# mjrgh/DCSExplorer

Measured on AMD Instinct MI355X. Metric: bit_exact_int16_pcm_samples_per_sec, higher is better.
Workload: dtype int16; 1 GPU; survey3_65536; gpu_max_hw_queues=4, samples_per_frame=240, frames_per_wave=8, wavefronts_per_launch=8192, arithmetic=ADSP-2105 1.15 fixed point, 32-bit integer intermediates, partition=range over streams, no collective, scale=1, inflight=1, frames_per_chunk=all, full=False

## Files before the change

dcsexplorer_amd/csrc/dcs_common.h:

```cpp
#pragma once
#include <stdint.h>
#include <stddef.h>
#include "../../include/dcs_hip.h"

#define DCS_CB94_TOTAL   940
#define DCS_TRIE94_MAX   64
#define DCS_TRIE93_MAX   128

struct DcsLdsTables
{
    uint16_t cb94[DCS_CB94_TOTAL];
    uint16_t fast93[256];
    uint16_t trie93[DCS_TRIE93_MAX];
    uint16_t bandBits93a[64];
    uint16_t scaleCb93a[80];
    uint8_t  inputs93a[24];
    uint16_t raw94[20];
    uint32_t band94[72];
    uint16_t scale64[64];
    uint8_t  padDecode_[8];
    uint16_t cbInfo[8];
    uint16_t xlat94[48];
    uint8_t  preAdj94[32];
    uint16_t scaleMant[4];
    uint8_t  pad_[8];
};
#define DCS_LDS_DECODE_BYTES 3424
#define DCS_B94_RAW      (1u << 21)
#define DCS_B94_ZERO     (1u << 22)
#define DCS_B94_STOP     (1u << 23)
#define DCS_B94_FATAL    (1u << 24)
#define DCS_B94_TYPE0    51

#define DCS_LANE_CONSTS 24
#define DCS_K94_PRE   0
#define DCS_K94_TWB   8
#define DCS_K94_OVLA  22
#define DCS_K94_OVLB  23
#define DCS_K93_TWB   0
#define DCS_K93_OVL   15

struct DcsDevTables
{
    DcsLdsTables lds;
    uint32_t lane94[64][DCS_LANE_CONSTS];
    uint32_t lane93[64][DCS_LANE_CONSTS];
    uint16_t fast94[256];
    uint16_t trie94[DCS_TRIE94_MAX];
    uint16_t pair93a[2048];
    uint16_t fftCoef[256];
    uint16_t ovlCoef[16];
    int32_t  twA[8][4];
    uint8_t  multi94[6][1 << 10];
};
#define DCS_IDX_MULTI_BITS 10
#define DCS_IDX_MULTI_SAMPLES 4

const DcsDevTables &dcsTables();

int dcsFrameScaleV(const uint16_t *vol, uint16_t *mixMul, const uint8_t *counted, int nch);

#define DCS_POOL_DW_PER_FRAME 56
#define DCS_POOL_DW_MIN       320
#define DCS_MAX_FRAME_BITS    4480

#ifdef __cplusplus
static inline
#ifdef __HIPCC__
__host__ __device__
#endif
uint32_t dcsPoolDwords(uint64_t streamOff, uint32_t hdrLen, uint32_t bitOff, uint32_t nBits)
{
    const uint32_t inDword = static_cast<uint32_t>(((streamOff + 2 + hdrLen) * 8 + bitOff) & 31);
    return (inDword + nBits + 31) / 32 + 3;
}
#endif

#ifdef __cplusplus
static inline
// ... 205 lines not shown
```

dcsexplorer_amd/csrc/dcs_decode_chunk.inc.h:

```cpp
    DCS_STAMP(1);

    struct { uint32_t job; uint32_t prevSlot, flags, nSrc, shiftXform; uint32_t firstSrc, prevJob, poolOff, bpl; } slot;
    uint32_t exportNext;
    uint4 pd0, pd1, phdr;
    uint2 pd2;
    {
        uint4 *scratch = reinterpret_cast<uint4 *>(L.pool());
        static_assert(kHeadVec * 16 <= poolDwords(FPW) * 4, "the package head fits in the bit pool");
        if (lane < kHeadVec)
            scratch[lane] = phead0;
        if (kHeadLoads > 1 && lane + 64 < kHeadVec)
            scratch[lane + 64] = phead1;
        waveSync();
        const uint4 *sp5 = scratch + 5 * s;
        const uint4 s0 = sp5[0];
        pd0 = sp5[1]; pd1 = sp5[2];
        const uint4 d2v = sp5[3];
        pd2 = make_uint2(d2v.x, d2v.y);
        phdr = sp5[4];
        waveSync();
        slot.job = s0.x;
        slot.prevSlot = s0.y & 0xFFu; slot.flags = (s0.y >> 8) & 0xFFu; slot.nSrc = (s0.y >> 16) & 0xFFu; slot.shiftXform = s0.y >> 24;
        slot.firstSrc = s0.z; slot.prevJob = s0.w;
        slot.poolOff = d2v.z & 0xFFFFu;
// ... 326 lines not shown
        }
        const int lpfShift = (xf == DCS_XFORM_94) ? 3 : 4;
        const int g = lane >> lpfShift;
        const bool active = g < n;
        const int mySlot = s0 + (active ? g : 0);
        const int myWord = __shfl(slotWord, mySlot);
        const int myFlags = myWord & 0xFF, myPrevSlot = (myWord >> 8) & 0xFF, myShift = myWord >> 16;
        const uint32_t myJob = static_cast<uint32_t>(__shfl(slotJob, mySlot));
        const uint32_t myPrevJob = static_cast<uint32_t>(__shfl(jobPrev, mySlot));
        const int lr = (xf == DCS_XFORM_94) ? bitrevN(lane & 7, 3) : bitrevN(lane & 15, 4);

        uint32_t extTail = 0;
        if (__any(active && (myFlags & DCS_SLOT_EXT_TAIL) != 0))
        {
            if (active && (myFlags & DCS_SLOT_EXT_TAIL) != 0 && a.tailsIn != nullptr)
            {
                const size_t k = static_cast<size_t>(myPrevJob & 0x7FFFFFFFu);
                extTail = (xf == DCS_XFORM_94) ? reinterpret_cast<const uint32_t *>(a.tailsIn)[k * 8 + lr]
                                               : static_cast<uint32_t>(static_cast<uint16_t>(a.tailsIn[k * 16 + lr]));
            }
        }

        PassLane P;
        P.rowC = active ? reinterpret_cast<uint32_t *>(L.row(mySlot)) : L.pool();
#ifdef DCS_STAMPS_XFORM
        P.stamp = stamp;
#endif
        P.l = lane & ((1 << lpfShift) - 1);
        P.shiftPair = static_cast<uint32_t>(myShift) * 0x00010001u;
        P.paced = paced && kPace.steps && s0 + n >= nSlots;

        uint32_t x[16];
        BflyRegs R;
        R.k8000 = 0x8000u; R.k10000 = 0x10000u; R.watch = 0xFFFFu;
        R.k4000 = 0x4000u; R.watchB = 0x7FFF7FFFu;
        asm volatile("" : "+v"(R.k8000), "+v"(R.k10000), "+v"(R.k4000));
        if (xf == DCS_XFORM_94)
            transform94x8<kPace.levels>(P, W, C, R, x);
        else
            transform93x4<kPace.levels>(P, W, C, R, x);
        if (s0 == 0) DCS_STAMP(14);

        {
            const int ts = active ? mySlot : FPW;
            if (xf == DCS_XFORM_94)
                tails[ts * 8 + lr] = x[15];
            else
                reinterpret_cast<uint16_t *>(tails)[ts * 16 + lr] = static_cast<uint16_t>(x[15]);
        }
        waveSync();

        if (s0 == 0) DCS_STAMP(15);
        const bool emit = active && !(myFlags & DCS_SLOT_HALO);
        const bool hasPrev = myPrevSlot != DCS_NO_PREV_SLOT;
        const bool exporter = active && (myFlags & DCS_SLOT_EXPORT) != 0;
        const bool deferred = active && (myFlags & DCS_SLOT_IMPORT) != 0;
#ifndef DCS_RDV_SPLIT_FPW4
#define DCS_RDV_SPLIT_FPW4 12
#endif
        constexpr int kSplit = FPW == 4 ? DCS_RDV_SPLIT_FPW4 : 8;
        int lrA = lr;
        if (FPW == 4)
            asm volatile("" : "+v"(lrA));
        unsigned long long metAsProducer = 0, metAsConsumer = 0;
        auto rendezvous = [&](uint32_t mine0, uint32_t tailOut)
        {
            if (exporter)
                metAsProducer = __hip_atomic_exchange(a.handoff + static_cast<size_t>(chunk) * 16 + lrA, handoffWord(a.epoch, 0u, tailOut),
                                                      __ATOMIC_RELAXED, __HIP_MEMORY_SCOPE_AGENT);
            if (deferred)
                metAsConsumer = __hip_atomic_exchange(a.handoff + static_cast<size_t>(myPrevJob) * 16 + lrA, handoffWord(a.epoch, 1u, mine0),
                                                      __ATOMIC_RELAXED, __HIP_MEMORY_SCOPE_AGENT);
        };
        if (xf == DCS_XFORM_94)
        {
            uint32_t tailPair = tails[(hasPrev ? myPrevSlot : mySlot) * 8 + lr];
            tailPair = hasPrev ? tailPair : extTail;
            const uint32_t mixed = packC(overlapMix(reC(x[0]), C.k[DCS_K94_OVLA] & 0xFFFFu, reC(tailPair), C.k[DCS_K94_OVLB] & 0xFFFFu),
                                         overlapMix(imC(x[0]), C.k[DCS_K94_OVLA] >> 16, imC(tailPair), C.k[DCS_K94_OVLB] >> 16));
            x[0] = deferred ? x[0] : mixed;
            uint32_t *out = reinterpret_cast<uint32_t *>(a.pcm) + static_cast<size_t>(myJob) * (DCS_FRAME_SAMPLES / 2) + lrA;
            if (emit)
            {
                if (!deferred)
                    out[0] = x[0];
#pragma unroll
                for (int r = 1 ; r < kSplit ; ++r)
                    out[8 * bitrevN(r, 4)] = x[r];
            }
            rendezvous(x[0], x[15]);
            if (emit)
            {
#pragma unroll
                for (int r = kSplit ; r < 15 ; ++r)
                    out[8 * bitrevN(r, 4)] = x[r];
                if (a.tailsOut != nullptr && (myFlags & DCS_SLOT_KEEP_TAIL))
// ... 52 lines not shown
```

dcsexplorer_amd/csrc/dcs_kernels.hip.h:

```cpp
#pragma once
#include <hip/hip_runtime.h>
#include <type_traits>
#include <cstddef>
#include "dcs_common.h"

namespace dcsk {

struct Stamper
{
#ifdef DCS_STAMPS
    unsigned long long *p;
#ifdef DCS_STAMPS_REALTIME
    __device__ __forceinline__ void operator()(int k) const { if (p != nullptr) p[k] = __builtin_amdgcn_s_memrealtime(); }
#else
    __device__ __forceinline__ void operator()(int k) const { if (p != nullptr) p[k] = __builtin_amdgcn_s_memtime(); }
#endif
#else
    __device__ __forceinline__ void operator()(int) const { }
#endif
};
#define DCS_STAMP(k) stamp(k)

__device__ __forceinline__ unsigned long long handoffWord(uint32_t epoch, uint32_t who, uint32_t payload)
{
// ... 643 lines not shown
    mr = odd ? mrOdd : mr;
    exponent = ((exponent + (odd ? 1 : 0)) >> 1) + 1;
    const uint32_t up = mr << (exponent & 31);
    const uint32_t down = static_cast<uint32_t>(static_cast<int>(mr) >> ((-exponent) & 31));
    uint32_t ar = (exponent >= 0 ? up : down) >> 16;
    ar = neg ? static_cast<uint32_t>(-sx16(ar)) & 0xFFFFu : ar;
    ar = x != 0 ? ar : 0u;
    *reinterpret_cast<uint32_t *>(row) = ar;
}

typedef short s16x2 __attribute__((ext_vector_type(2)));
typedef unsigned short u16x2 __attribute__((ext_vector_type(2)));

__device__ __forceinline__ uint32_t pkAddSat(uint32_t a, uint32_t b)
{ return __builtin_bit_cast(uint32_t, __builtin_elementwise_add_sat(__builtin_bit_cast(s16x2, a), __builtin_bit_cast(s16x2, b))); }
__device__ __forceinline__ uint32_t pkSubSat(uint32_t a, uint32_t b)
{ return __builtin_bit_cast(uint32_t, __builtin_elementwise_sub_sat(__builtin_bit_cast(s16x2, a), __builtin_bit_cast(s16x2, b))); }
__device__ __forceinline__ uint32_t pkAdd(uint32_t a, uint32_t b)
{ return __builtin_bit_cast(uint32_t, static_cast<u16x2>(__builtin_bit_cast(u16x2, a) + __builtin_bit_cast(u16x2, b))); }
__device__ __forceinline__ uint32_t pkSub(uint32_t a, uint32_t b)
{ return __builtin_bit_cast(uint32_t, static_cast<u16x2>(__builtin_bit_cast(u16x2, a) - __builtin_bit_cast(u16x2, b))); }
__device__ __forceinline__ uint32_t pkAshr(uint32_t a, uint32_t shiftPair)
{ return __builtin_bit_cast(uint32_t, static_cast<s16x2>(__builtin_bit_cast(s16x2, a) >> __builtin_bit_cast(s16x2, shiftPair))); }

__device__ __forceinline__ uint32_t packC(int re, int im) { return (static_cast<uint32_t>(re) & 0xFFFFu) | (static_cast<uint32_t>(im) << 16); }
__device__ __forceinline__ int reC(uint32_t c) { return sx16(c); }
__device__ __forceinline__ int imC(uint32_t c) { return static_cast<int>(c) >> 16; }

__device__ __forceinline__ void quirkWatch(uint32_t &watch, uint32_t a, uint32_t b)
{
    asm("v_min_u16 %0, %0, %1\n\tv_min_u16 %0, %0, %2" : "+v"(watch) : "v"(a), "v"(b));
}
__device__ __forceinline__ bool quirkSeen(uint32_t watch) { return __any((watch & 0xFFFFu) == 0); }
#define DCS_MUL_SEL(dst, x, xsel, y, ysel) \
    asm("v_mul_i32_i24_sdwa %0, sext(%1), sext(%2) dst_sel:DWORD dst_unused:UNUSED_PAD src0_sel:" xsel " src1_sel:" ysel : "=v"(dst) : "v"(x), "v"(y))

struct BflyRegs
{
    uint32_t k8000, k10000; uint32_t watch;
    uint32_t k4000, watchB;
};

struct TwScalar { int c2, s2, ns2; };
struct TwA { TwScalar t[8]; };
constexpr int kTwADoubled[8][2] = { { -65536, 0 }, { 0, -65536 }, { -46340, -46340 }, { 46340, -46340 },
                                    { -60548, -25080 }, { 25080, -60548 }, { -25080, -60548 }, { 60548, -25080 } };
__device__ __forceinline__ void loadTwA(const DcsDevTables *, TwA &W)
{
#pragma unroll
    for (int k = 2 ; k < 8 ; ++k)
        W.t[k] = TwScalar{ kTwADoubled[k][0], kTwADoubled[k][1], -kTwADoubled[k][1] };
}

__device__ __forceinline__ uint32_t rotateExact(uint32_t A, int c, int s)
{
    const int are = reC(A), aim = imC(A);
    const int p2 = __mul24(aim, s);
    const int dR = __mul24(are, c) - p2;
    const int q2 = __mul24(are, s);
    const int dI = __mul24(aim, c) + q2;
    uint32_t mrR = (static_cast<uint32_t>(dR) << 1) + 0x8000u;
    uint32_t mrI = (static_cast<uint32_t>(dI) << 1) + 0x8000u;
    if ((p2 & 0x7FFF) == 0x4000) mrR &= ~0x10000u;
    if ((q2 & 0x7FFF) == 0x4000) mrI &= ~0x10000u;
    return __builtin_amdgcn_perm(mrI, mrR, 0x07060302u);
}

__device__ __forceinline__ uint32_t rotateFastA(uint32_t A, const TwScalar &t, BflyRegs &R)
{
    const int are = reC(A), aim = imC(A);
    const uint32_t nP = static_cast<uint32_t>(__mul24(aim, t.ns2)) + R.k8000;
    const uint32_t mrR = static_cast<uint32_t>(__mul24(are, t.c2)) + nP;
    const uint32_t qK = static_cast<uint32_t>(__mul24(are, t.s2)) + R.k8000;
    const uint32_t mrI = static_cast<uint32_t>(__mul24(aim, t.c2)) + qK;
    quirkWatch(R.watch, nP, qK);
    return __builtin_amdgcn_perm(mrI, mrR, 0x07060302u);
}
__device__ __forceinline__ uint32_t shl1Add(uint32_t a, uint32_t b)
{
    uint32_t r = (a << 1) + b;
    asm("" : "+v"(r));
    return r;
}
template <bool TIGHT>
__device__ __forceinline__ uint32_t rotateFastB(uint32_t A, uint32_t tw, BflyRegs &R)
{
    int p1, p2, q1, q2;
    DCS_MUL_SEL(p2, A, "WORD_1", tw, "WORD_1");
    DCS_MUL_SEL(p1, A, "WORD_0", tw, "WORD_0");
    DCS_MUL_SEL(q2, A, "WORD_0", tw, "WORD_1");
    DCS_MUL_SEL(q1, A, "WORD_1", tw, "WORD_0");
    if (TIGHT)
    {
        const uint32_t tR = shl1Add(static_cast<uint32_t>(p2), R.k8000);
        const uint32_t mrR = shl1Add(static_cast<uint32_t>(p1), R.k10000) - tR;
        const uint32_t qK = shl1Add(static_cast<uint32_t>(q2), R.k8000);
        const uint32_t mrI = shl1Add(static_cast<uint32_t>(q1), qK);
        quirkWatch(R.watch, tR, qK);
        return __builtin_amdgcn_perm(mrI, mrR, 0x07060302u);
    }
    const uint32_t mrR = (static_cast<uint32_t>(p1 - p2) << 1) + R.k8000;
    const uint32_t qK = (static_cast<uint32_t>(q2) << 1) + R.k8000;
    const uint32_t mrI = (static_cast<uint32_t>(q1) << 1) + qK;
    quirkWatch(R.watch, (static_cast<uint32_t>(p2) << 1) + R.k8000, qK);
    return __builtin_amdgcn_perm(mrI, mrR, 0x07060302u);
}

struct TwDot { uint32_t re, im, s2; };
__device__ __forceinline__ TwDot deriveTwDot(uint32_t tw)
{
    TwDot d;
    d.im = __builtin_amdgcn_alignbit(tw, tw, 16);
    d.re = __builtin_bit_cast(uint32_t, static_cast<u16x2>(__builtin_bit_cast(u16x2, tw) * __builtin_bit_cast(u16x2, 0xFFFF0001u)));
    asm("v_pk_add_u16 %0, %1, %1 op_sel:[1,1] op_sel_hi:[1,1]" : "=v"(d.s2) : "v"(tw));
    return d;
}
template <bool FIX>
__device__ __forceinline__ uint32_t rotateDotB(uint32_t A, const TwDot &t, BflyRegs &R, uint32_t fixMask)
{
    uint32_t xR, xI, lows;
    const uint32_t cR = FIX ? ((A & fixMask) | R.k4000) : R.k4000;
    asm("v_dot2_i32_i16 %0, %1, %2, %3" : "=v"(xR) : "v"(A), "v"(t.re), "v"(cR));
    asm("v_dot2_i32_i16 %0, %1, %2, %3" : "=v"(xI) : "v"(A), "v"(t.im), "v"(R.k4000));
    asm("v_pk_mul_lo_u16 %0, %1, %2" : "=v"(lows) : "v"(A), "v"(t.s2));
    asm("v_pk_min_i16 %0, %0, %1" : "+v"(R.watchB) : "v"(lows));
    return __builtin_amdgcn_perm(xI << 1, xR << 1, 0x07060302u);
}
__device__ __forceinline__ bool quirkSeenB(uint32_t w) { return __any((w & 0xFFFFu) == 0x8000u || (w >> 16) == 0x8000u); }

template <bool SAT>
__device__ __forceinline__ void addSub(uint32_t u, uint32_t T, uint32_t &lo, uint32_t &hi)
{
    if (SAT) { lo = pkSubSat(u, T); hi = pkAddSat(u, T); }
    else     { lo = pkSub(u, T);    hi = pkAdd(u, T); }
}

__device__ __forceinline__ uint32_t rotateByMinusOne(uint32_t A) { return pkSub(0u, A); }
__device__ __forceinline__ uint32_t rotateByMinusI(uint32_t A)
{
    return __builtin_bit_cast(uint32_t, static_cast<u16x2>(__builtin_bit_cast(u16x2, __builtin_amdgcn_alignbit(A, A, 16))
                                                            * __builtin_bit_cast(u16x2, 0xFFFF0001u)));
}

template <bool SAT, int D, int SH>
__device__ __forceinline__ void stageA(uint32_t (&x)[16], const TwA &W, BflyRegs &R)
{
    uint32_t y[16];
#pragma unroll
    for (int r = 0 ; r < 16 ; ++r)
        if (!(r & D))
        {
            const int idx = r >> SH;
            const uint32_t T = idx == 0 ? rotateByMinusOne(x[r + D]) : idx == 1 ? rotateByMinusI(x[r + D])
                                                                                 : rotateFastA(x[r + D], W.t[idx], R);
            addSub<SAT>(x[r], T, y[r], y[r + D]);
        }
    if (__builtin_expect(quirkSeen(R.watch), 0))
    {
        R.watch = 0xFFFFu;
#pragma unroll
        for (int r = 0 ; r < 16 ; ++r)
            if (!(r & D) && (r >> SH) >= 2)
            {
                int c2 = W.t[r >> SH].c2, s2 = W.t[r >> SH].s2;
                asm volatile("" : "+v"(c2), "+v"(s2));
                addSub<SAT>(x[r], rotateExact(x[r + D], c2 >> 1, s2 >> 1), y[r], y[r + D]);
            }
    }
#pragma unroll
    for (int r = 0 ; r < 16 ; ++r)
        x[r] = y[r];
}
template <bool SAT, int D, int SH, bool DOT = !SAT>
__device__ __forceinline__ void stageB(uint32_t (&x)[16], const uint32_t *tw, BflyRegs &R)
{
    uint32_t y[16];
    bool redo;
    if constexpr (DOT)
    {
        constexpr int kTw = 8 / D;
        TwDot td[kTw];
#pragma unroll
        for (int k = 0 ; k < kTw ; ++k)
            td[k] = deriveTwDot(tw[k]);
        constexpr int kFix = kTw == 1 ? 0 : 1;
        const uint32_t fixMask = tw[kFix] == 0x80000000u ? 0xFFFF0000u : 0u;
#pragma unroll
        for (int r = 0 ; r < 16 ; ++r)
            if (!(r & D))
            {
                const uint32_t T = (r >> SH) == kFix ? rotateDotB<true>(x[r + D], td[r >> SH], R, fixMask)
                                                     : rotateDotB<false>(x[r + D], td[r >> SH], R, 0u);
                addSub<SAT>(x[r], T, y[r], y[r + D]);
            }
        redo = quirkSeenB(R.watchB);
        if (redo)
            R.watchB = 0x7FFF7FFFu;
    }
    else
    {
#pragma unroll
        for (int r = 0 ; r < 16 ; ++r)
            if (!(r & D))
                addSub<SAT>(x[r], rotateFastB<SAT>(x[r + D], tw[r >> SH], R), y[r], y[r + D]);
        redo = quirkSeen(R.watch);
        if (redo)
            R.watch = 0xFFFFu;
    }
    if (__builtin_expect(redo, 0))
    {
#pragma unroll
        for (int r = 0 ; r < 16 ; ++r)
            if (!(r & D))
                addSub<SAT>(x[r], rotateExact(x[r + D], sx16(tw[r >> SH]), static_cast<int>(tw[r >> SH]) >> 16), y[r], y[r + D]);
    }
#pragma unroll
    for (int r = 0 ; r < 16 ; ++r)
        x[r] = y[r];
}

__device__ __forceinline__ int bitrev9(int v) { return static_cast<int>(__brev(static_cast<uint32_t>(v)) >> 23); }
__device__ __forceinline__ int bitrevN(int v, int bits) { return static_cast<int>(__brev(static_cast<uint32_t>(v)) >> (32 - bits)); }

__device__ __forceinline__ int overlapMix(int x, uint32_t cx, int o, uint32_t co)
{
    const uint32_t a = static_cast<uint32_t>(x * static_cast<int>(cx)) << 1;
    const uint32_t b = static_cast<uint32_t>(o * static_cast<int>(co)) << 1;
    return static_cast<int>(a + b + 0x8000u) >> 16;
}

typedef uint32_t u32x4a4 __attribute__((ext_vector_type(4), aligned(4)));

struct LaneConsts { uint32_t k[DCS_LANE_CONSTS]; };
__device__ __forceinline__ void loadLaneConsts(const DcsDevTables *G, int lane, int xform, LaneConsts &C)
{
    const uint4 *src = reinterpret_cast<const uint4 *>(xform == DCS_XFORM_94 ? G->lane94[lane] : G->lane93[lane]);
#pragma unroll
    for (int i = 0 ; i < DCS_LANE_CONSTS / 4 ; ++i)
    {
        const uint4 v = src[i];
        C.k[4 * i] = v.x; C.k[4 * i + 1] = v.y; C.k[4 * i + 2] = v.z; C.k[4 * i + 3] = v.w;
    }
}

__device__ __forceinline__ void waveSync()
{
    __builtin_amdgcn_fence(__ATOMIC_RELEASE, "wavefront");
    __builtin_amdgcn_wave_barrier();
    __builtin_amdgcn_fence(__ATOMIC_ACQUIRE, "wavefront");
}

struct PassLane
{
    uint32_t *rowC;
    int l;
    uint32_t shiftPair;
    bool paced;
#ifdef DCS_STAMPS_XFORM
    Stamper stamp;
#endif
};
constexpr int kPaceSteps = 2 | (1 << 2) | (0 << 4);
#define DCS_PACE_STEP(k) do { if (P.paced) __builtin_amdgcn_s_setprio((STEPS >> (2 * (k))) & 3); } while (0)
#ifdef DCS_STAMPS_XFORM
#define DCS_XSTAMP(k) P.stamp(k)
#else
#define DCS_XSTAMP(k)
#endif

__device__ __forceinline__ uint4 ldsRead4(const uint32_t *p) { return *reinterpret_cast<const uint4 *>(p); }
__device__ __forceinline__ void ldsWrite4(uint32_t *p, uint32_t a, uint32_t b, uint32_t c, uint32_t d)
{ *reinterpret_cast<uint4 *>(p) = make_uint4(a, b, c, d); }

__device__ __forceinline__ int swzQuad(int row, int quad) { return row * 16 + ((quad ^ (row >> 1)) & 3) * 4; }
__device__ __forceinline__ int swzPos(int row, int pos) { return swzQuad(row, pos >> 2) + (pos & 3); }

template <int STEPS>
__device__ __forceinline__ void transform94x8(const PassLane &P, const TwA &W, const LaneConsts &C, BflyRegs &R, uint32_t (&x)[16])
{
    const int l = P.l;
    uint32_t *S = P.rowC;
    uint32_t An[8], Bn[8];
    {
        uint32_t a_[8], b_[8];
#pragma unroll
        for (int j = 0 ; j < 8 ; ++j)
        {
            const int i = l + 8 * j;
            const uint32_t X = P.rowC[i];
            uint32_t Y = P.rowC[(128 - i) & 127];
            if (i == 0) Y = 0;
            const uint32_t Sm = pkAddSat(X, Y), Df = pkSubSat(X, Y);
            a_[j] = pkSub(0u, __builtin_amdgcn_perm(Df, Sm, 0x07060100u));
            b_[j] = pkSub(0u, __builtin_amdgcn_perm(Sm, Df, 0x07060100u));
        }
        auto finish = [&](int j, uint32_t Pr)
        {
            const uint32_t a = a_[j];
            An[j] = pkAddSat(Pr, a);
            const uint32_t t = pkSubSat(a, Pr);
            const uint32_t t2 = pkSubSat(Pr, a);
            Bn[j] = __builtin_amdgcn_perm(t2, t, 0x07060100u);
        };
#pragma unroll
        for (int j = 0 ; j < 8 ; ++j)
        {
            int p1, p2, q1, q2;
            DCS_MUL_SEL(p2, b_[j], "WORD_0", C.k[DCS_K94_PRE + j], "WORD_0");
            DCS_MUL_SEL(p1, b_[j], "WORD_1", C.k[DCS_K94_PRE + j], "WORD_1");
            DCS_MUL_SEL(q2, b_[j], "WORD_0", C.k[DCS_K94_PRE + j], "WORD_1");
            DCS_MUL_SEL(q1, b_[j], "WORD_1", C.k[DCS_K94_PRE + j], "WORD_0");
            const uint32_t tR = shl1Add(static_cast<uint32_t>(p2), R.k8000);
            const uint32_t m0 = shl1Add(static_cast<uint32_t>(p1), R.k10000) - tR;
            const uint32_t qK = shl1Add(static_cast<uint32_t>(q2), R.k8000);
            const uint32_t m1 = shl1Add(static_cast<uint32_t>(q1), qK);
            quirkWatch(R.watch, tR, qK);
            finish(j, __builtin_amdgcn_perm(m0, m1, 0x07060302u));
        }
        if (__builtin_expect(quirkSeen(R.watch), 0))
        {
            R.watch = 0xFFFFu;
#pragma unroll
            for (int j = 0 ; j < 8 ; ++j)
            {
                const int b0 = reC(b_[j]), b1 = imC(b_[j]);
                const int c0 = sx16(C.k[DCS_K94_PRE + j]), c1 = static_cast<int>(C.k[DCS_K94_PRE + j]) >> 16;
                const int p2 = __mul24(b0, c0), q2 = __mul24(b0, c1);
                uint32_t m0 = (static_cast<uint32_t>(__mul24(b1, c1) - p2) << 1) + 0x8000u;
                uint32_t m1 = (static_cast<uint32_t>(__mul24(b1, c0) + q2) << 1) + 0x8000u;
                if ((p2 & 0x7FFF) == 0x4000) m0 &= ~0x10000u;
                if ((q2 & 0x7FFF) == 0x4000) m1 &= ~0x10000u;
                finish(j, __builtin_amdgcn_perm(m0, m1, 0x07060302u));
            }
        }
    }
    if (l == 0)
    {
        const uint32_t M = P.rowC[64];
        Bn[0] = __builtin_amdgcn_perm(M, pkSub(0u, M), 0x07060100u);
    }
    waveSync();
    {
        ldsWrite4(S + swzQuad(l, 0), An[0], An[1], An[2], An[3]);
        ldsWrite4(S + swzQuad(l, 1), An[4], An[5], An[6], An[7]);
        const int rb = (8 - l) & 7;
        if (l != 0)
        {
            ldsWrite4(S + swzQuad(rb, 2), Bn[7], Bn[6], Bn[5], Bn[4]);
            ldsWrite4(S + swzQuad(rb, 3), Bn[3], Bn[2], Bn[1], Bn[0]);
        }
        else
        {
            ldsWrite4(S + swzQuad(rb, 2), Bn[0], Bn[7], Bn[6], Bn[5]);
            ldsWrite4(S + swzQuad(rb, 3), Bn[4], Bn[3], Bn[2], Bn[1]);
        }
    }
    waveSync();
#pragma unroll
    for (int c = 0 ; c < 4 ; ++c)
    {
        const uint4 v = ldsRead4(S + swzQuad(l, c));
        x[4 * c] = v.x; x[4 * c + 1] = v.y; x[4 * c + 2] = v.z; x[4 * c + 3] = v.w;
    }
    waveSync();
    DCS_PACE_STEP(0);
#pragma unroll
    for (int r = 0 ; r < 8 ; ++r)
    {
        const uint32_t u = x[r], a = x[r + 8];
        x[r] = pkAddSat(u, a); x[r + 8] = pkSubSat(u, a);
    }
    stageA<true, 4, 3>(x, W, R);
    stageA<true, 2, 2>(x, W, R);
    stageA<true, 1, 1>(x, W, R);
    DCS_PACE_STEP(1);
#pragma unroll
    for (int r = 0 ; r < 16 ; ++r)
        S[swzPos(r >> 1, 8 * (r & 1) + l)] = x[r];
    waveSync();
#pragma unroll
    for (int c = 0 ; c < 4 ; ++c)
    {
        const uint4 v = ldsRead4(S + swzQuad(l, c));
        x[4 * c] = v.x; x[4 * c + 1] = v.y; x[4 * c + 2] = v.z; x[4 * c + 3] = v.w;
    }
    stageB<true, 4, 3>(x, C.k + DCS_K94_TWB, R);
    DCS_PACE_STEP(2);
    stageB<true, 2, 2>(x, C.k + DCS_K94_TWB + 2, R);
    stageB<true, 1, 1>(x, C.k + DCS_K94_TWB + 6, R);
    if (__any(P.shiftPair != 0))
    {
#pragma unroll
        for (int r = 0 ; r < 16 ; ++r)
            x[r] = pkAshr(x[r], P.shiftPair);
    }
}

template <int STEPS>
__device__ __forceinline__ void transform93x4(const PassLane &P, const TwA &W, const LaneConsts &C, BflyRegs &R, uint32_t (&x)[16])
{
    const int l = P.l;
    uint32_t *S = P.rowC;
#pragma unroll
    for (int r = 0 ; r < 8 ; ++r)
    {
        const int p = 16 * r + l;
        const uint32_t A = P.rowC[p];
        const uint32_t B = P.rowC[(128 - p) & 127];
        const uint32_t Sm = pkAdd(A, B), Df = pkSub(A, B);
        x[r] = __builtin_amdgcn_perm(Df, Sm, 0x07060100u);
        x[r + 8] = __builtin_amdgcn_perm(Sm, Df, 0x07060100u);
        if (p == 0)
        {
            x[0] = A; x[8] = A;
        }
    }
    DCS_XSTAMP(8);
    DCS_PACE_STEP(0);
    stageA<false, 4, 3>(x, W, R);
    stageA<false, 2, 2>(x, W, R);
    stageA<false, 1, 1>(x, W, R);
    DCS_XSTAMP(9);
    waveSync();
    uint32_t y[16];
#pragma unroll
    for (int h = 0 ; h < 2 ; ++h)
    {
#pragma unroll
        for (int r = 0 ; r < 8 ; ++r)
            S[swzPos(r, l)] = x[8 * h + r];
        waveSync();
        if ((l >> 3) == h)
        {
#pragma unroll
            for (int c = 0 ; c < 4 ; ++c)
            {
                const uint4 v = ldsRead4(S + swzQuad(l & 7, c));
                y[4 * c] = v.x; y[4 * c + 1] = v.y; y[4 * c + 2] = v.z; y[4 * c + 3] = v.w;
            }
        }
        waveSync();
    }
#pragma unroll
    for (int r = 0 ; r < 16 ; ++r)
        x[r] = y[r];
    DCS_XSTAMP(10);
    DCS_PACE_STEP(1);
    stageB<false, 8, 4>(x, C.k + DCS_K93_TWB, R);
    stageB<false, 4, 3>(x, C.k + DCS_K93_TWB + 1, R);
    DCS_PACE_STEP(2);
    stageB<false, 2, 2>(x, C.k + DCS_K93_TWB + 3, R);
    stageB<false, 1, 1>(x, C.k + DCS_K93_TWB + 7, R);
    DCS_XSTAMP(11);
    if (__any(P.shiftPair != 0))
    {
#pragma unroll
        for (int r = 0 ; r < 16 ; ++r)
            x[r] = pkAshr(x[r], P.shiftPair);
    }
}

#ifndef DCS_CPW2_SCHED
#define DCS_CPW2_SCHED 1
#endif
struct PaceSchedule { int entry; bool steps; int levels; };
__host__ __device__ constexpr PaceSchedule paceSchedule(int cpw, int pass)
{
    if (cpw == 1)
        return { 3, true, kPaceSteps };
#if DCS_CPW2_SCHED == 0
    return pass == 0 ? PaceSchedule{ 3, false, kPaceSteps } : PaceSchedule{ 3, true, 2 | (1 << 2) | (0 << 4) };
#elif DCS_CPW2_SCHED == 1
    return pass == 0 ? PaceSchedule{ 3, false, kPaceSteps } : PaceSchedule{ 2, true, 1 | (1 << 2) | (0 << 4) };
#elif DCS_CPW2_SCHED == 2
    return pass == 0 ? PaceSchedule{ 3, true, 3 | (3 << 2) | (2 << 4) } : PaceSchedule{ 2, true, 1 | (1 << 2) | (0 << 4) };
#else
    return pass == 0 ? PaceSchedule{ 3, true, 3 | (2 << 2) | (2 << 4) } : PaceSchedule{ 1, true, 1 | (0 << 2) | (0 << 4) };
#endif
}

template <int FPW, int CPW = 1>
#ifndef DCS_MIN_WAVES
#define DCS_MIN_WAVES 4
#endif
__global__ void __launch_bounds__(64 * kWavesPerBlock, DCS_MIN_WAVES)
// ... 138 lines not shown
```

dcsexplorer_amd/csrc/dcs_tables.cpp:

```cpp
#include <cstddef>
#include "dcs_common.h"
#include "dcs_tables.h"
#include <stdlib.h>
#include <string.h>
#include <vector>

namespace {

template <size_t N, typename F>
void buildVlc(const DcsVlc (&codes)[N], uint16_t *fast, uint16_t *trie, size_t trieCap, F payload)
{
    struct Node { int child[2]; int leaf; };
    std::vector<Node> nodes;
    nodes.push_back({{-1, -1}, -1});
    for (const DcsVlc &c : codes)
    {
        int n = 0;
        for (int b = c.len - 1 ; b >= 0 ; --b)
        {
            int bit = (c.code >> b) & 1;
            if (nodes[n].child[bit] < 0)
            {
                nodes[n].child[bit] = static_cast<int>(nodes.size());
                nodes.push_back({{-1, -1}, -1});
// ... 135 lines not shown
        t.lds.band94[k] = static_cast<uint32_t>(book) | ((shPeek & 31u) << 11) | ((shIdx & 31u) << 16) | (raw ? DCS_B94_RAW : 0u)
                        | (zero ? DCS_B94_ZERO : 0u) | (stop ? DCS_B94_STOP : 0u) | (fatal ? DCS_B94_FATAL : 0u) | (adj << 25);
    }
    memcpy(t.lds.bandBits93a, kBandBits93a, sizeof(t.lds.bandBits93a));
    memcpy(t.lds.scaleCb93a, kScaleCb93a, sizeof(t.lds.scaleCb93a));
    for (int i = 0 ; i < 18 ; ++i)
        t.lds.inputs93a[i] = kInputsPerBand93a[i];
    memcpy(t.lds.scaleMant, kScaleMant, sizeof(t.lds.scaleMant));
    for (int c = 0 ; c < 64 ; ++c)
        t.lds.scale64[c] = static_cast<uint16_t>(kScaleMant[c & 3] >> (15 - ((c >> 2) & 15)));
    if (kScaleMant[0] != 0x8000 || kScaleMant[1] != 0x9838 || kScaleMant[2] != 0xB505 || kScaleMant[3] != 0xD745)
        abort();
    memcpy(t.pair93a, kPair93a, sizeof(t.pair93a));
    memcpy(t.fftCoef, kFftCoef, sizeof(t.fftCoef));
    if (kFftCoef[0x80] != 0x8000 || kFftCoef[0] != 0x0000 || kFftCoef[0x81] != 0x0000 || kFftCoef[1] != 0x8000)
        abort();
    memcpy(t.ovlCoef, kOverlapCoef, sizeof(t.ovlCoef));
    static const int kTwAInKernel[8][2] = { { -65536, 0 }, { 0, -65536 }, { -46340, -46340 }, { 46340, -46340 },
                                            { -60548, -25080 }, { 25080, -60548 }, { -25080, -60548 }, { 60548, -25080 } };
    for (int k = 0 ; k < 8 ; ++k)
    {
        const int c = static_cast<int16_t>(kFftCoef[0x80 + k]), sn = static_cast<int16_t>(kFftCoef[k]);
        t.twA[k][0] = 2 * c; t.twA[k][1] = 2 * sn; t.twA[k][2] = -2 * sn; t.twA[k][3] = 0;
        if (kTwAInKernel[k][0] != 2 * c || kTwAInKernel[k][1] != 2 * sn)
            abort();
    }

    auto rev = [](int v, int bits) { int r = 0; for (int i = 0 ; i < bits ; ++i) r |= ((v >> i) & 1) << (bits - 1 - i); return r; };
    auto tw = [&](int part) { return static_cast<uint32_t>(kFftCoef[0x80 + part]) | (static_cast<uint32_t>(kFftCoef[part]) << 16); };
    for (int lane = 0 ; lane < 64 ; ++lane)
    {
        uint32_t *k94 = t.lane94[lane], *k93 = t.lane93[lane];
        const int l8 = lane & 7, l16 = lane & 15;
        for (int j = 0 ; j < 8 ; ++j)
        {
            const int i = l8 + 8 * j;
            k94[DCS_K94_PRE + j] = static_cast<uint32_t>(kFftCoef[rev(2 + 4 * i, 9)]) | (static_cast<uint32_t>(kFftCoef[rev(4 * i, 9)]) << 16);
        }
        for (int k = 0 ; k < 2 ; ++k) k94[DCS_K94_TWB + k] = tw(2 * l8 + k);
        for (int k = 0 ; k < 4 ; ++k) k94[DCS_K94_TWB + 2 + k] = tw(4 * l8 + k);
        for (int k = 0 ; k < 8 ; ++k) k94[DCS_K94_TWB + 6 + k] = tw(8 * l8 + k);
        k93[DCS_K93_TWB] = tw(l16);
        for (int k = 0 ; k < 2 ; ++k) k93[DCS_K93_TWB + 1 + k] = tw(2 * l16 + k);
        for (int k = 0 ; k < 4 ; ++k) k93[DCS_K93_TWB + 3 + k] = tw(4 * l16 + k);
        for (int k = 0 ; k < 8 ; ++k) k93[DCS_K93_TWB + 7 + k] = tw(8 * l16 + k);
        const int m = rev(l8, 3);
        k94[DCS_K94_OVLA] = static_cast<uint32_t>(kOverlapCoef[2 * m]) | (static_cast<uint32_t>(kOverlapCoef[2 * m + 1]) << 16);
        k94[DCS_K94_OVLB] = static_cast<uint32_t>(kOverlapCoef[15 - 2 * m]) | (static_cast<uint32_t>(kOverlapCoef[14 - 2 * m]) << 16);
        const int i = rev(l16, 4);
        k93[DCS_K93_OVL] = static_cast<uint32_t>(kOverlapCoef[i]) | (static_cast<uint32_t>(kOverlapCoef[15 - i]) << 16);
    }
    return t;
}

}

const DcsDevTables &dcsTables()
{
    static const DcsDevTables tables = build();
    return tables;
}

static_assert(sizeof(DcsLdsTables) % 16 == 0, "LDS table block must be a multiple of 16 bytes");
static_assert(DCS_LDS_DECODE_BYTES % 16 == 0 && DCS_LDS_DECODE_BYTES == offsetof(DcsLdsTables, cbInfo), "the decode kernel stages the block up to the index walk's tables");
static_assert(offsetof(DcsDevTables, lane94) % 16 == 0 && offsetof(DcsDevTables, lane93) % 16 == 0 && offsetof(DcsDevTables, twA) % 16 == 0, "lane constants and twiddles are fetched as uint4");
static_assert(sizeof(DcsSrcDesc) == 160, "DcsSrcDesc layout");
static_assert(offsetof(DcsSrcDesc, idx) == 12, "DcsSrcDesc layout");
static_assert(sizeof(DcsFrameJob) == 16, "DcsFrameJob layout");
static_assert(sizeof(DcsFrameIndex) == 148 && offsetof(DcsFrameIndex, split) == 28, "DcsFrameIndex layout");
static_assert(sizeof(DcsSlot) == 32, "DcsSlot layout");
static_assert(offsetof(DcsDevTables, pair93a) % 4 == 0, "OS93a sample pairs are read as 32-bit words");
```

Baseline: 507.3 billion samples/s.

## Use dot2 rotations with precomputed twiddle triples for 1994 transform stages

Replaces the four SDWA 24-bit multiplies per complex rotation in the 1994+ pre-twiddle and butterfly stages with two v_dot2_i32_i16 ops plus a packed low-word check. The needed coefficients come from a new per-lane global table of (re, im, 2*sin) triples, loaded in pieces just before each stage. Shrinking the per-lane constant block lets a register go. The rare saturation quirk is caught by a packed-min watch and triggers an exact redo, and one fixed lane/twiddle pair gets a correction mask. This trades ALU work for more global loads and added register pressure from the staged triples.

```diff
diff --git a/dcsexplorer_amd/csrc/dcs_common.h b/dcsexplorer_amd/csrc/dcs_common.h
--- a/dcsexplorer_amd/csrc/dcs_common.h
+++ b/dcsexplorer_amd/csrc/dcs_common.h
@@ -32,19 +32,25 @@
 #define DCS_B94_FATAL    (1u << 24)
 #define DCS_B94_TYPE0    51
 
-#define DCS_LANE_CONSTS 24
-#define DCS_K94_PRE   0
-#define DCS_K94_TWB   8
-#define DCS_K94_OVLA  22
-#define DCS_K94_OVLB  23
+#define DCS_LANE_CONSTS 16
+#define DCS_K94_OVLA  0
+#define DCS_K94_OVLB  1
 #define DCS_K93_TWB   0
 #define DCS_K93_OVL   15
+#define DCS_D94_PRE    0
+#define DCS_D94_S4     24
+#define DCS_D94_S2     32
+#define DCS_D94_S1     44
+#define DCS_D94_DWORDS 68
+#define DCS_D94_FIX_TW 1
+#define DCS_D94_FIX_PRE 0
 
 struct DcsDevTables
 {
     DcsLdsTables lds;
     uint32_t lane94[64][DCS_LANE_CONSTS];
     uint32_t lane93[64][DCS_LANE_CONSTS];
+    uint32_t dot94[8][DCS_D94_DWORDS];
     uint16_t fast94[256];
     uint16_t trie94[DCS_TRIE94_MAX];
     uint16_t pair93a[2048];
diff --git a/dcsexplorer_amd/csrc/dcs_decode_chunk.inc.h b/dcsexplorer_amd/csrc/dcs_decode_chunk.inc.h
--- a/dcsexplorer_amd/csrc/dcs_decode_chunk.inc.h
+++ b/dcsexplorer_amd/csrc/dcs_decode_chunk.inc.h
@@ -382,11 +382,11 @@
 
         uint32_t x[16];
         BflyRegs R;
-        R.k8000 = 0x8000u; R.k10000 = 0x10000u; R.watch = 0xFFFFu;
+        R.k8000 = 0x8000u; R.watch = 0xFFFFu;
         R.k4000 = 0x4000u; R.watchB = 0x7FFF7FFFu;
-        asm volatile("" : "+v"(R.k8000), "+v"(R.k10000), "+v"(R.k4000));
+        asm volatile("" : "+v"(R.k8000), "+v"(R.k4000));
         if (xf == DCS_XFORM_94)
-            transform94x8<kPace.levels>(P, W, C, R, x);
+            transform94x8<kPace.levels>(P, W, a.tables, R, x);
         else
             transform93x4<kPace.levels>(P, W, C, R, x);
         if (s0 == 0) DCS_STAMP(14);
@@ -410,8 +410,7 @@
 #endif
         constexpr int kSplit = FPW == 4 ? DCS_RDV_SPLIT_FPW4 : 8;
         int lrA = lr;
-        if (FPW == 4)
-            asm volatile("" : "+v"(lrA));
+        asm volatile("" : "+v"(lrA));
         unsigned long long metAsProducer = 0, metAsConsumer = 0;
         auto rendezvous = [&](uint32_t mine0, uint32_t tailOut)
         {
diff --git a/dcsexplorer_amd/csrc/dcs_kernels.hip.h b/dcsexplorer_amd/csrc/dcs_kernels.hip.h
--- a/dcsexplorer_amd/csrc/dcs_kernels.hip.h
+++ b/dcsexplorer_amd/csrc/dcs_kernels.hip.h
@@ -699,12 +699,9 @@
     asm("v_min_u16 %0, %0, %1\n\tv_min_u16 %0, %0, %2" : "+v"(watch) : "v"(a), "v"(b));
 }
 __device__ __forceinline__ bool quirkSeen(uint32_t watch) { return __any((watch & 0xFFFFu) == 0); }
-#define DCS_MUL_SEL(dst, x, xsel, y, ysel) \
-    asm("v_mul_i32_i24_sdwa %0, sext(%1), sext(%2) dst_sel:DWORD dst_unused:UNUSED_PAD src0_sel:" xsel " src1_sel:" ysel : "=v"(dst) : "v"(x), "v"(y))
-
 struct BflyRegs
 {
-    uint32_t k8000, k10000; uint32_t watch;
+    uint32_t k8000; uint32_t watch;
     uint32_t k4000, watchB;
 };
 
@@ -743,36 +740,6 @@
     quirkWatch(R.watch, nP, qK);
     return __builtin_amdgcn_perm(mrI, mrR, 0x07060302u);
 }
-__device__ __forceinline__ uint32_t shl1Add(uint32_t a, uint32_t b)
-{
-    uint32_t r = (a << 1) + b;
-    asm("" : "+v"(r));
-    return r;
-}
-template <bool TIGHT>
-__device__ __forceinline__ uint32_t rotateFastB(uint32_t A, uint32_t tw, BflyRegs &R)
-{
-    int p1, p2, q1, q2;
-    DCS_MUL_SEL(p2, A, "WORD_1", tw, "WORD_1");
-    DCS_MUL_SEL(p1, A, "WORD_0", tw, "WORD_0");
-    DCS_MUL_SEL(q2, A, "WORD_0", tw, "WORD_1");
-    DCS_MUL_SEL(q1, A, "WORD_1", tw, "WORD_0");
-    if (TIGHT)
-    {
-        const uint32_t tR = shl1Add(static_cast<uint32_t>(p2), R.k8000);
-        const uint32_t mrR = shl1Add(static_cast<uint32_t>(p1), R.k10000) - tR;
-        const uint32_t qK = shl1Add(static_cast<uint32_t>(q2), R.k8000);
-        const uint32_t mrI = shl1Add(static_cast<uint32_t>(q1), qK);
-        quirkWatch(R.watch, tR, qK);
-        return __builtin_amdgcn_perm(mrI, mrR, 0x07060302u);
-    }
-    const uint32_t mrR = (static_cast<uint32_t>(p1 - p2) << 1) + R.k8000;
-    const uint32_t qK = (static_cast<uint32_t>(q2) << 1) + R.k8000;
-    const uint32_t mrI = (static_cast<uint32_t>(q1) << 1) + qK;
-    quirkWatch(R.watch, (static_cast<uint32_t>(p2) << 1) + R.k8000, qK);
-    return __builtin_amdgcn_perm(mrI, mrR, 0x07060302u);
-}
-
 struct TwDot { uint32_t re, im, s2; };
 __device__ __forceinline__ TwDot deriveTwDot(uint32_t tw)
 {
@@ -838,52 +805,91 @@
     for (int r = 0 ; r < 16 ; ++r)
         x[r] = y[r];
 }
-template <bool SAT, int D, int SH, bool DOT = !SAT>
-__device__ __forceinline__ void stageB(uint32_t (&x)[16], const uint32_t *tw, BflyRegs &R)
+template <bool SAT, int D, int SH, int RLO, int RHI>
+__device__ __forceinline__ void bflysDotB(const uint32_t (&x)[16], uint32_t (&y)[16], const TwDot *td, int kFix, BflyRegs &R, uint32_t fixMask)
+{
+#pragma unroll
+    for (int r = RLO ; r < RHI ; ++r)
+        if (!(r & D))
+        {
+            const TwDot &t = td[(r >> SH) - (RLO >> SH)];
+            const uint32_t T = (r >> SH) == kFix ? rotateDotB<true>(x[r + D], t, R, fixMask) : rotateDotB<false>(x[r + D], t, R, 0u);
+            addSub<SAT>(x[r], T, y[r], y[r + D]);
+        }
+}
+template <int D, int SH>
+__device__ __forceinline__ void stageB93(uint32_t (&x)[16], const uint32_t *tw, BflyRegs &R)
 {
     uint32_t y[16];
-    bool redo;
-    if constexpr (DOT)
-    {
-        constexpr int kTw = 8 / D;
-        TwDot td[kTw];
-#pragma unroll
-        for (int k = 0 ; k < kTw ; ++k)
-            td[k] = deriveTwDot(tw[k]);
-        constexpr int kFix = kTw == 1 ? 0 : 1;
-        const uint32_t fixMask = tw[kFix] == 0x80000000u ? 0xFFFF0000u : 0u;
+    constexpr int kTw = 8 / D;
+    TwDot td[kTw];
+#pragma unroll
+    for (int k = 0 ; k < kTw ; ++k)
+        td[k] = deriveTwDot(tw[k]);
+    constexpr int kFix = kTw == 1 ? 0 : 1;
+    const uint32_t fixMask = tw[kFix] == 0x80000000u ? 0xFFFF0000u : 0u;
+    bflysDotB<false, D, SH, 0, 16>(x, y, td, kFix, R, fixMask);
+    if (__builtin_expect(quirkSeenB(R.watchB), 0))
+    {
+        R.watchB = 0x7FFF7FFFu;
 #pragma unroll
         for (int r = 0 ; r < 16 ; ++r)
             if (!(r & D))
-            {
-                const uint32_t T = (r >> SH) == kFix ? rotateDotB<true>(x[r + D], td[r >> SH], R, fixMask)
-                                                     : rotateDotB<false>(x[r + D], td[r >> SH], R, 0u);
-                addSub<SAT>(x[r], T, y[r], y[r + D]);
-            }
-        redo = quirkSeenB(R.watchB);
-        if (redo)
-            R.watchB = 0x7FFF7FFFu;
-    }
-    else
-    {
-#pragma unroll
-        for (int r = 0 ; r < 16 ; ++r)
-            if (!(r & D))
-                addSub<SAT>(x[r], rotateFastB<SAT>(x[r + D], tw[r >> SH], R), y[r], y[r + D]);
-        redo = quirkSeen(R.watch);
-        if (redo)
-            R.watch = 0xFFFFu;
-    }
-    if (__builtin_expect(redo, 0))
-    {
-#pragma unroll
-        for (int r = 0 ; r < 16 ; ++r)
-            if (!(r & D))
-                addSub<SAT>(x[r], rotateExact(x[r + D], sx16(tw[r >> SH]), static_cast<int>(tw[r >> SH]) >> 16), y[r], y[r + D]);
+                addSub<false>(x[r], rotateExact(x[r + D], sx16(tw[r >> SH]), static_cast<int>(tw[r >> SH]) >> 16), y[r], y[r + D]);
     }
 #pragma unroll
     for (int r = 0 ; r < 16 ; ++r)
         x[r] = y[r];
+}
+
+template <int N>
+__device__ __forceinline__ void loadDot94(const DcsDevTables *G, uint32_t rowOff, int part, TwDot (&t)[N])
+{
+    static_assert(N % 2 == 0, "whole 8-byte pieces");
+    const char *row = reinterpret_cast<const char *>(G->dot94) + rowOff;
+    uint32_t w[3 * N];
+#pragma unroll
+    for (int i = 0 ; i < 3 * N / 4 ; ++i)
+    {
+        const uint4 v = reinterpret_cast<const uint4 *>(row + 4 * part)[i];
+        w[4 * i] = v.x; w[4 * i + 1] = v.y; w[4 * i + 2] = v.z; w[4 * i + 3] = v.w;
+    }
+    if constexpr ((3 * N) % 4 != 0)
+    {
+        const uint2 v = *reinterpret_cast<const uint2 *>(row + 4 * (part + 3 * N - 2));
+        w[3 * N - 2] = v.x; w[3 * N - 1] = v.y;
+    }
+#pragma unroll
+    for (int k = 0 ; k < N ; ++k)
+        t[k] = TwDot{ w[3 * k], w[3 * k + 1], w[3 * k + 2] };
+}
+__device__ __forceinline__ uint32_t loadDot94Sc(const DcsDevTables *G, uint32_t rowOff, int part, int k)
+{
+    return *reinterpret_cast<const uint32_t *>(reinterpret_cast<const char *>(G->dot94) + rowOff + 4 * (part + 3 * k + 1));
+}
+__device__ __forceinline__ uint32_t lanePos0Mul(int l)
+{
+    uint32_t z = static_cast<uint32_t>(l);
+    asm volatile("" : "+v"(z));
+    return (min(z, 1u) ^ 1u) << 16;
+}
+__device__ __forceinline__ uint32_t dot94Row(uint32_t rowOff, uint32_t &after)
+{
+    asm volatile("" : "+v"(rowOff), "+v"(after));
+    return rowOff;
+}
+template <int D, int SH>
+__device__ __forceinline__ void redoStage94(const uint32_t (&x)[16], uint32_t (&y)[16], const DcsDevTables *G, uint32_t rowOff, int part)
+{
+    constexpr int kTw = 8 / D;
+    uint32_t sc[kTw];
+#pragma unroll
+    for (int k = 0 ; k < kTw ; ++k)
+        sc[k] = loadDot94Sc(G, rowOff, part, k);
+#pragma unroll
+    for (int r = 0 ; r < 16 ; ++r)
+        if (!(r & D))
+            addSub<true>(x[r], rotateExact(x[r + D], static_cast<int>(sc[r >> SH]) >> 16, sx16(sc[r >> SH])), y[r], y[r + D]);
 }
 
 __device__ __forceinline__ int bitrev9(int v) { return static_cast<int>(__brev(static_cast<uint32_t>(v)) >> 23); }
@@ -943,10 +949,14 @@
 __device__ __forceinline__ int swzPos(int row, int pos) { return swzQuad(row, pos >> 2) + (pos & 3); }
 
 template <int STEPS>
-__device__ __forceinline__ void transform94x8(const PassLane &P, const TwA &W, const LaneConsts &C, BflyRegs &R, uint32_t (&x)[16])
+__device__ __forceinline__ void transform94x8(const PassLane &P, const TwA &W, const DcsDevTables *G, BflyRegs &R, uint32_t (&x)[16])
 {
     const int l = P.l;
     uint32_t *S = P.rowC;
+    uint32_t rowOff = static_cast<uint32_t>(l) * (DCS_D94_DWORDS * 4u);
+    TwDot pre[8];
+    asm volatile("" : "+v"(rowOff));
+    loadDot94<8>(G, rowOff, DCS_D94_PRE, pre);
     uint32_t An[8], Bn[8];
     {
         uint32_t a_[8], b_[8];
@@ -969,29 +979,29 @@
             const uint32_t t2 = pkSubSat(Pr, a);
             Bn[j] = __builtin_amdgcn_perm(t2, t, 0x07060100u);
         };
+        const uint32_t fixMul = lanePos0Mul(l);
 #pragma unroll
         for (int j = 0 ; j < 8 ; ++j)
         {
-            int p1, p2, q1, q2;
-            DCS_MUL_SEL(p2, b_[j], "WORD_0", C.k[DCS_K94_PRE + j], "WORD_0");
-            DCS_MUL_SEL(p1, b_[j], "WORD_1", C.k[DCS_K94_PRE + j], "WORD_1");
-            DCS_MUL_SEL(q2, b_[j], "WORD_0", C.k[DCS_K94_PRE + j], "WORD_1");
-            DCS_MUL_SEL(q1, b_[j], "WORD_1", C.k[DCS_K94_PRE + j], "WORD_0");
-            const uint32_t tR = shl1Add(static_cast<uint32_t>(p2), R.k8000);
-            const uint32_t m0 = shl1Add(static_cast<uint32_t>(p1), R.k10000) - tR;
-            const uint32_t qK = shl1Add(static_cast<uint32_t>(q2), R.k8000);
-            const uint32_t m1 = shl1Add(static_cast<uint32_t>(q1), qK);
-            quirkWatch(R.watch, tR, qK);
-            finish(j, __builtin_amdgcn_perm(m0, m1, 0x07060302u));
-        }
-        if (__builtin_expect(quirkSeen(R.watch), 0))
-        {
-            R.watch = 0xFFFFu;
+            uint32_t x0, x1, lows;
+            const uint32_t c0 = j == DCS_D94_FIX_PRE ? __umul24(b_[j], fixMul) + R.k4000 : R.k4000;
+            asm("v_dot2_i32_i16 %0, %1, %2, %3" : "=v"(x0) : "v"(b_[j]), "v"(pre[j].re), "v"(c0));
+            asm("v_dot2_i32_i16 %0, %1, %2, %3" : "=v"(x1) : "v"(b_[j]), "v"(pre[j].im), "v"(R.k4000));
+            asm("v_pk_mul_lo_u16 %0, %1, %2 op_sel:[0,0] op_sel_hi:[0,1]" : "=v"(lows) : "v"(b_[j]), "v"(pre[j].s2));
+            asm("v_pk_min_i16 %0, %0, %1" : "+v"(R.watchB) : "v"(lows));
+            finish(j, __builtin_amdgcn_perm(x0 << 1, x1 << 1, 0x07060302u));
+        }
+        if (__builtin_expect(quirkSeenB(R.watchB), 0))
+        {
+            R.watchB = 0x7FFF7FFFu;
+            uint32_t ro = rowOff;
+            asm volatile("" : "+v"(ro));
 #pragma unroll
             for (int j = 0 ; j < 8 ; ++j)
             {
                 const int b0 = reC(b_[j]), b1 = imC(b_[j]);
-                const int c0 = sx16(C.k[DCS_K94_PRE + j]), c1 = static_cast<int>(C.k[DCS_K94_PRE + j]) >> 16;
+                const uint32_t cc = loadDot94Sc(G, ro, DCS_D94_PRE, j);
+                const int c1 = sx16(cc), c0 = static_cast<int>(cc) >> 16;
                 const int p2 = __mul24(b0, c0), q2 = __mul24(b0, c1);
                 uint32_t m0 = (static_cast<uint32_t>(__mul24(b1, c1) - p2) << 1) + 0x8000u;
                 uint32_t m1 = (static_cast<uint32_t>(__mul24(b1, c0) + q2) << 1) + 0x8000u;
@@ -1041,6 +1051,12 @@
     stageA<true, 2, 2>(x, W, R);
     stageA<true, 1, 1>(x, W, R);
     DCS_PACE_STEP(1);
+    TwDot t4[2], t2[4];
+    {
+        const uint32_t ro = dot94Row(rowOff, x[0]);
+        loadDot94<2>(G, ro, DCS_D94_S4, t4);
+        loadDot94<4>(G, ro, DCS_D94_S2, t2);
+    }
 #pragma unroll
     for (int r = 0 ; r < 16 ; ++r)
         S[swzPos(r >> 1, 8 * (r & 1) + l)] = x[r];
@@ -1051,10 +1067,36 @@
         const uint4 v = ldsRead4(S + swzQuad(l, c));
         x[4 * c] = v.x; x[4 * c + 1] = v.y; x[4 * c + 2] = v.z; x[4 * c + 3] = v.w;
     }
-    stageB<true, 4, 3>(x, C.k + DCS_K94_TWB, R);
+    const uint32_t fixMask = 0u - lanePos0Mul(l);
+    auto stage = [&](auto dTag, auto shTag, int part, auto &&bflys)
+    {
+        constexpr int D = decltype(dTag)::value, SH = decltype(shTag)::value;
+        uint32_t y[16];
+        bflys(y);
+        if (__builtin_expect(quirkSeenB(R.watchB), 0))
+        {
+            R.watchB = 0x7FFF7FFFu;
+            uint32_t ro = rowOff;
+            asm volatile("" : "+v"(ro));
+            redoStage94<D, SH>(x, y, G, ro, part);
+        }
+#pragma unroll
+        for (int r = 0 ; r < 16 ; ++r)
+            x[r] = y[r];
+    };
+    using I1 = std::integral_constant<int, 1>; using I2 = std::integral_constant<int, 2>;
+    using I3 = std::integral_constant<int, 3>; using I4 = std::integral_constant<int, 4>;
+    stage(I4{}, I3{}, DCS_D94_S4, [&](uint32_t (&y)[16]) { bflysDotB<true, 4, 3, 0, 16>(x, y, t4, DCS_D94_FIX_TW, R, fixMask); });
     DCS_PACE_STEP(2);
-    stageB<true, 2, 2>(x, C.k + DCS_K94_TWB + 2, R);
-    stageB<true, 1, 1>(x, C.k + DCS_K94_TWB + 6, R);
+    TwDot t1a[4], t1b[4];
+    loadDot94<4>(G, dot94Row(rowOff, x[0]), DCS_D94_S1, t1a);
+    stage(I2{}, I2{}, DCS_D94_S2, [&](uint32_t (&y)[16]) { bflysDotB<true, 2, 2, 0, 16>(x, y, t2, DCS_D94_FIX_TW, R, fixMask); });
+    loadDot94<4>(G, dot94Row(rowOff, x[0]), DCS_D94_S1 + 12, t1b);
+    stage(I1{}, I1{}, DCS_D94_S1, [&](uint32_t (&y)[16])
+    {
+        bflysDotB<true, 1, 1, 0, 8>(x, y, t1a, DCS_D94_FIX_TW, R, fixMask);
+        bflysDotB<true, 1, 1, 8, 16>(x, y, t1b, DCS_D94_FIX_TW, R, fixMask);
+    });
     if (__any(P.shiftPair != 0))
     {
 #pragma unroll
@@ -1113,11 +1155,11 @@
         x[r] = y[r];
     DCS_XSTAMP(10);
     DCS_PACE_STEP(1);
-    stageB<false, 8, 4>(x, C.k + DCS_K93_TWB, R);
-    stageB<false, 4, 3>(x, C.k + DCS_K93_TWB + 1, R);
+    stageB93<8, 4>(x, C.k + DCS_K93_TWB, R);
+    stageB93<4, 3>(x, C.k + DCS_K93_TWB + 1, R);
     DCS_PACE_STEP(2);
-    stageB<false, 2, 2>(x, C.k + DCS_K93_TWB + 3, R);
-    stageB<false, 1, 1>(x, C.k + DCS_K93_TWB + 7, R);
+    stageB93<2, 2>(x, C.k + DCS_K93_TWB + 3, R);
+    stageB93<1, 1>(x, C.k + DCS_K93_TWB + 7, R);
     DCS_XSTAMP(11);
     if (__any(P.shiftPair != 0))
     {
diff --git a/dcsexplorer_amd/csrc/dcs_tables.cpp b/dcsexplorer_amd/csrc/dcs_tables.cpp
--- a/dcsexplorer_amd/csrc/dcs_tables.cpp
+++ b/dcsexplorer_amd/csrc/dcs_tables.cpp
@@ -191,14 +191,6 @@
     {
         uint32_t *k94 = t.lane94[lane], *k93 = t.lane93[lane];
         const int l8 = lane & 7, l16 = lane & 15;
-        for (int j = 0 ; j < 8 ; ++j)
-        {
-            const int i = l8 + 8 * j;
-            k94[DCS_K94_PRE + j] = static_cast<uint32_t>(kFftCoef[rev(2 + 4 * i, 9)]) | (static_cast<uint32_t>(kFftCoef[rev(4 * i, 9)]) << 16);
-        }
-        for (int k = 0 ; k < 2 ; ++k) k94[DCS_K94_TWB + k] = tw(2 * l8 + k);
-        for (int k = 0 ; k < 4 ; ++k) k94[DCS_K94_TWB + 2 + k] = tw(4 * l8 + k);
-        for (int k = 0 ; k < 8 ; ++k) k94[DCS_K94_TWB + 6 + k] = tw(8 * l8 + k);
         k93[DCS_K93_TWB] = tw(l16);
         for (int k = 0 ; k < 2 ; ++k) k93[DCS_K93_TWB + 1 + k] = tw(2 * l16 + k);
         for (int k = 0 ; k < 4 ; ++k) k93[DCS_K93_TWB + 3 + k] = tw(4 * l16 + k);
@@ -209,6 +201,40 @@
         const int i = rev(l16, 4);
         k93[DCS_K93_OVL] = static_cast<uint32_t>(kOverlapCoef[i]) | (static_cast<uint32_t>(kOverlapCoef[15 - i]) << 16);
     }
+
+    auto pk = [](uint32_t lo, uint32_t hi) { return (lo & 0xFFFFu) | (hi << 16); };
+    auto putTw = [&](uint32_t *d, uint32_t packed)
+    {
+        const uint32_t c = packed & 0xFFFFu, sn = packed >> 16;
+        d[0] = pk(c, 0u - sn); d[1] = pk(sn, c); d[2] = pk(2 * sn, 2 * sn);
+        if ((d[1] >> 16 | d[1] << 16) != packed || static_cast<uint16_t>(d[0]) != c
+            || static_cast<uint16_t>((d[0] >> 16) + sn) != 0 || static_cast<uint16_t>(d[2]) != static_cast<uint16_t>(sn + sn) || (d[2] >> 16) != (d[2] & 0xFFFFu))
+            abort();
+        return sn == 0x8000u;
+    };
+    for (int l8 = 0 ; l8 < 8 ; ++l8)
+    {
+        uint32_t *d = t.dot94[l8];
+        for (int j = 0 ; j < 8 ; ++j)
+        {
+            const int i = l8 + 8 * j;
+            const uint32_t c0 = kFftCoef[rev(2 + 4 * i, 9)], c1 = kFftCoef[rev(4 * i, 9)];
+            uint32_t *e = d + DCS_D94_PRE + 3 * j;
+            e[0] = pk(0u - c0, c1); e[1] = pk(c1, c0); e[2] = pk(2 * c0, 2 * c1);
+            if ((c0 == 0x8000u) != (l8 == 0 && j == DCS_D94_FIX_PRE))
+                abort();
+            if (static_cast<uint16_t>((e[0] & 0xFFFFu) + c0) != 0 || (e[0] >> 16) != c1 || (e[1] >> 16) != c0 || (e[1] & 0xFFFFu) != c1)
+                abort();
+        }
+        for (int k = 0 ; k < 2 ; ++k)
+            if (putTw(d + DCS_D94_S4 + 3 * k, tw(2 * l8 + k)) != (l8 == 0 && k == DCS_D94_FIX_TW)) abort();
+        for (int k = 0 ; k < 4 ; ++k)
+            if (putTw(d + DCS_D94_S2 + 3 * k, tw(4 * l8 + k)) != (l8 == 0 && k == DCS_D94_FIX_TW)) abort();
+        for (int k = 0 ; k < 8 ; ++k)
+            if (putTw(d + DCS_D94_S1 + 3 * k, tw(8 * l8 + k)) != (l8 == 0 && k == DCS_D94_FIX_TW)) abort();
+    }
+    if (tw(1) != 0x80000000u)
+        abort();
     return t;
 }
 
@@ -220,8 +246,21 @@
     return tables;
 }
 
+extern "C" uint32_t dcs_debug_dot94(uint32_t *dot94, uint16_t *fftCoef)
+{
+    const DcsDevTables &t = dcsTables();
+    if (dot94 != nullptr)
+        memcpy(dot94, t.dot94, sizeof(t.dot94));
+    if (fftCoef != nullptr)
+        memcpy(fftCoef, t.fftCoef, sizeof(t.fftCoef));
+    return DCS_D94_DWORDS;
+}
+
 static_assert(sizeof(DcsLdsTables) % 16 == 0, "LDS table block must be a multiple of 16 bytes");
 static_assert(DCS_LDS_DECODE_BYTES % 16 == 0 && DCS_LDS_DECODE_BYTES == offsetof(DcsLdsTables, cbInfo), "the decode kernel stages the block up to the index walk's tables");
+static_assert(offsetof(DcsDevTables, dot94) % 16 == 0 && (DCS_D94_DWORDS % 4) == 0 && (DCS_D94_S4 % 4) == 0 && (DCS_D94_S2 % 4) == 0 && (DCS_D94_S1 % 4) == 0
+              && DCS_D94_S4 == DCS_D94_PRE + 24 && DCS_D94_S2 >= DCS_D94_S4 + 6 && DCS_D94_S1 == DCS_D94_S2 + 12 && DCS_D94_DWORDS == DCS_D94_S1 + 24,
+              "the 1994+ twiddle triples are fetched as uint4, part by part");
 static_assert(offsetof(DcsDevTables, lane94) % 16 == 0 && offsetof(DcsDevTables, lane93) % 16 == 0 && offsetof(DcsDevTables, twA) % 16 == 0, "lane constants and twiddles are fetched as uint4");
 static_assert(sizeof(DcsSrcDesc) == 160, "DcsSrcDesc layout");
 static_assert(offsetof(DcsSrcDesc, idx) == 12, "DcsSrcDesc layout");
```

After: 494.1 billion samples/s. -2.6%, worse.
